# SheffieldML/GPy

Hardware: AMD Instinct MI355X
Metric: exact-GP log_lik+grad iters/sec (higher is better)
Workload: dtype f64; 1 GPU; BASELINE configs[2]: matern52 ARD exact GP, one GPRegression.parameters_changed, N=16384 D=32 Dy=1 per GPU; N=16384, D=32, kernel=matern52, ARD=True, parallelism=replicas x1

## Files before the change

gpy_amd/_lib.py:

```python
import ctypes
import os
import subprocess

import numpy as np
from numpy.ctypeslib import ndpointer

_HERE = os.path.dirname(os.path.abspath(__file__))
LIB_PATH = os.environ.get("MI355GP_LIB") or os.path.join(_HERE, "libmi355gp.so")
CSRC = os.path.join(_HERE, "csrc")

KIND_IDS = {"rbf": 0, "matern52": 1, "matern32": 2, "exponential": 3, "white": 4, "bias": 5, "ratquad": 6, "stdperiodic": 7,
            "coregionalize": 8, "linear": 9, "mlp": 10, "poly": 11, "cosine": 12, "sinc": 13, "expquadcosine": 14}


def ard_id(kind, ARD):
    if kind == "coregionalize":
        return int(ARD)
    return int(ARD) & 3 if kind == "stdperiodic" else int(bool(ARD))


class Part(ctypes.Structure):
    _fields_ = [("kind", ctypes.c_int), ("ard", ctypes.c_int), ("n_active", ctypes.c_int),
                ("active_dims", ctypes.POINTER(ctypes.c_int)), ("theta", ctypes.POINTER(ctypes.c_double)),
                ("term", ctypes.c_int)]


def make_parts(specs):
    arr = (Part * len(specs))()
    keep, ntheta = [], 0
    for i, spec in enumerate(specs):
        kind, ARD, theta, dims = spec[:4]
        arr[i].term = int(spec[4]) if len(spec) > 4 else 0
        th = np.ascontiguousarray(theta, dtype=np.float64)
        keep.append(th)
        arr[i].kind = KIND_IDS[kind]
        arr[i].ard = ard_id(kind, ARD)
        arr[i].theta = th.ctypes.data_as(ctypes.POINTER(ctypes.c_double))
        if dims is None:
            arr[i].n_active = 0
            arr[i].active_dims = None
        else:
            d = np.ascontiguousarray(dims, dtype=np.int32)
            keep.append(d)
            arr[i].n_active = d.size
            arr[i].active_dims = d.ctypes.data_as(ctypes.POINTER(ctypes.c_int))
        ntheta += th.size
    return arr, keep, ntheta
FETCH_L, FETCH_KINV, FETCH_DLDK, FETCH_K = 0, 1, 2, 3
EP_BERNOULLI_PROBIT = 0
OUT_LML, OUT_LOGDET, OUT_DATAFIT, OUT_DNOISE, OUT_TRKINV, NUM_OUT = 0, 1, 2, 3, 4, 8
STAGE_NAMES = ("kbuild", "potrf", "trtri", "lauum", "solve", "grad", "total")
NUM_T = 8
PROFILE_FAMILIES = ("update_nt", "trtri", "lauum", "diag128", "trsm128", "update_nt64", "potrf_persist", "trtri_early")

_lib = None


class MI355GPError(RuntimeError):
    pass


DIAG_LIB_PATH = os.path.join(_HERE, "libmi355gp_diag.so")


def build(force=False):
    srcs = [os.path.join(CSRC, f) for f in os.listdir(CSRC) if f.endswith((".hip", ".h")) or f == "Makefile"]
    srcs.append(os.path.join(_HERE, "..", "include", "mi355gp.h"))
    srcs.append(os.path.join(_HERE, "..", "include", "mi355gp_debug.h"))
    product = os.path.join(_HERE, "libmi355gp.so")
    if not force and os.path.exists(product) and os.path.exists(DIAG_LIB_PATH):
        t = min(os.path.getmtime(product), os.path.getmtime(DIAG_LIB_PATH))
        if all(os.path.getmtime(s) <= t for s in srcs if os.path.exists(s)):
            return product
    r = subprocess.run(["make", "-C", CSRC, "-j8", "all", "diag"], capture_output=True, text=True)
    if r.returncode != 0 or not os.path.exists(product) or not os.path.exists(DIAG_LIB_PATH):
        raise MI355GPError("building libmi355gp.so failed:\n" + r.stdout[-4000:] + r.stderr[-4000:])
    return product


_ci, _i64, _cd, _vp, _str = ctypes.c_int, ctypes.c_int64, ctypes.c_double, ctypes.c_void_p, ctypes.c_char_p
_dp = ndpointer(dtype=np.float64, flags="C_CONTIGUOUS")
_c_dp = ctypes.POINTER(ctypes.c_double)
_ip, _hp, _parts = ctypes.POINTER(_ci), ctypes.POINTER(_vp), ctypes.POINTER(Part)
_i32a, _i64a = (ndpointer(dtype=t, flags="C_CONTIGUOUS") for t in (np.int32, np.int64))
_EXACT = [_vp, _ci, _ci, _dp, _dp, _i64, _cd, _cd, _dp] + [_c_dp] * 4
_KERN_X2 = [_dp, _i64, _c_dp, _i64, _ci, _dp]

ABI = {
    "mi355gp_last_error": [],
    "mi355gp_version": [],
    "mi355gp_device_count": [_ip],
    "mi355gp_device_synchronize": [_ci],
    "mi355gp_create": [_ci, _hp],
    "mi355gp_destroy": [_vp],
    "mi355gp_set_data": [_vp, _dp, _i64, _ci, _dp, _ci],
    "mi355gp_set_targets": [_vp, _dp, _ci],
    "mi355gp_kern_K": [_ci, _ci, _ci, _dp] + _KERN_X2,
    "mi355gp_kern_Kdiag": [_ci, _dp, _i64, _dp],
    "mi355gp_update_gradients_full": [_ci, _ci, _ci, _dp, _dp] + _KERN_X2,
    "mi355gp_gradients_X": [_ci, _ci, _ci, _dp, _dp] + _KERN_X2,
    "mi355gp_exact_inference": _EXACT,
    "mi355gp_exact_inference_sum": [_vp, _ci, _parts, _dp, _i64, _cd, _cd, _dp] + [_c_dp] * 4,
    "mi355gp_exact_studentt_sum": [_vp, _ci, _parts, _cd, _cd, _cd, _dp] + [_c_dp] * 3,
    "mi355gp_inference_given_K": [_vp, _dp, _dp, _i64, _cd, _cd, _dp] + [_c_dp] * 3,
    "mi355gp_fetch": [_vp, _ci, _dp, _ci],
    "mi355gp_predict": [_vp, _ci, _ci, _dp, _dp, _i64, _c_dp, _c_dp, _ci],
    "mi355gp_predict_sum": [_vp, _ci, _parts, _dp, _i64, _c_dp, _c_dp, _ci],
    "mi355gp_predictive_gradients_sum": [_vp, _ci, _parts, _dp, _i64, _c_dp, _c_dp],
    "mi355gp_laplace_begin": [_vp, _ci, _parts],
    "mi355gp_laplace_newton": [_vp, _dp, _dp, _cd, _dp, _dp, _c_dp],
    "mi355gp_laplace_finish": [_vp, _dp, _cd, _dp, _c_dp],
    "mi355gp_laplace_gradients": [_vp, _dp, _dp, _dp],
    "mi355gp_laplace_implicit": [_vp, _dp, _dp],
    "mi355gp_laplace_predict": [_vp, _ci, _parts, _dp, _i64, _dp, _c_dp, _c_dp, _ci],
    "mi355gp_ep_recompute": [_vp, _dp, _dp, _cd, _cd, _ci, _dp, _dp, _c_dp, _c_dp],
    "mi355gp_ep_sweep": [_vp, _ci, _i64a, _dp, _cd, _cd] + [_dp] * 7 + [_c_dp],
    "mi355gp_covariance_between_points": [_vp, _ci, _parts, _dp, _i64, _dp, _i64, _dp],
    "mi355gp_potrf": [_ci, _dp, _i64, _c_dp],
    "mi355gp_pdinv": [_ci, _dp, _i64] + [_c_dp] * 4,
    "mi355gp_pdinv_full": [_ci, _dp, _i64] + [_c_dp] * 5,
    "mi355gp_set_option": [_vp, _ci, _ci],
    "mi355gp_get_option": [_vp, _ci, _ip],
    "mi355gp_get_profile": [_vp, _dp, _dp, _i32a],
    "mi355gp_grid_unique_id": [_str],
    "mi355gp_grid_create": [_ci] * 6 + [_str, _hp],
    "mi355gp_grid_destroy": [_vp],
    "mi355gp_grid_set_data": [_vp, _dp, _i64, _ci, _dp, _ci],
    "mi355gp_grid_exact_inference": _EXACT,
    "mi355gp_grid_fetch": [_vp, _ci, _dp],
    "mi355gp_grid_set_option": [_vp, _ci, _ci],
    "mi355gp_grid_get_option": [_vp, _ci, _ip],
    "mi355gp_grid_coll_log": [_vp, _ci, _dp],
    "mi355gp_sparse_create": [_ci, _hp],
    "mi355gp_sparse_destroy": [_vp],
    "mi355gp_sparse_set_data": [_vp, _dp, _i64, _ci, _dp, _ci],
    "mi355gp_vardtc_inference": _EXACT,
    "mi355gp_vardtc_inference_sum": [_vp, _ci, _parts, _dp, _i64, _dp, _i64, _cd, _dp] + [_c_dp] * 6,
    "mi355gp_sparse_set_input_variance": [_vp, _dp, _i64, _ci],
    "mi355gp_sparse_set_inputs": [_vp, _dp, _c_dp, _i64, _ci],
    "mi355gp_vardtc_inference_uncertain": [_vp, _ci, _parts, _dp, _i64, _dp, _i64, _cd, _dp] + [_c_dp] * 6,
    "mi355gp_sparse_predict": [_vp, _ci, _parts, _dp, _i64, _c_dp, _c_dp, _ci],
    "mi355gp_sparse_predict_uncertain": [_vp, _ci, _parts, _dp, _dp, _i64, _dp, _c_dp],
    "mi355gp_sparse_get_predict_ms": [_vp, _c_dp],
    "mi355gp_sparse_fetch_dLdKnm": [_vp, _i64, _i64, _dp],
    "mi355gp_sparse_attach_comm": [_vp, _ci, _ci, _str],
    "mi355gp_sparse_attach_loopback": [_vp, _ci, _ci, _ci],
    "mi355gp_sparse_fetch": [_vp, _ci, _dp],
    "mi355gp_sparse_get_profile": [_vp, _dp],
    "mi355gp_svgp_forward": [_vp, _ci, _parts, _dp, _i64, _dp, _dp, _ci, _cd, _dp, _dp, _dp, _c_dp],
    "mi355gp_svgp_backward": [_vp, _dp, _dp] + [_c_dp] * 5,
    "mi355gp_svgp_predict": [_vp, _ci, _parts, _c_dp, _i64, _ci] + [_c_dp] * 4,
    "mi355gp_pep_inference": [_vp, _ci, _parts, _dp, _i64, _cd, _cd, _cd, _dp] + [_c_dp] * 5,
    "mi355gp_pep_check_sigma": [_dp, _i64, _i64, _cd, _cd],
    "mi355gp_rbf_psi": [_ci, _cd, _dp, _ci, _dp, _i64, _dp, _dp, _i64, _ci] + [_c_dp] * 3,
    "mi355gp_rbf_psi_grad": [_ci, _cd, _dp, _ci, _dp, _i64, _dp, _dp, _i64, _ci] + [_c_dp] * 4 + [_dp] * 5,
    "mi355gp_bench_factor": [_ci, _i64, _ci, _c_dp, _c_dp, _c_dp],
    "mi355gp_dbg_ipc_selftest": [_str, _ci, _ci, _ci, _ci, _i64, _dp],
    "mi355gp_dbg_comm_selftest": [_ci, _str, _ci, _ci, _ci, _ci, _i64, _ci, _dp],
    "mi355gp_dbg_grid_multi": [_ci, _ci, _ci, _ci, _dp],
    "mi355gp_dbg_update_nt": [_ci, _ci, _ip, _ci, _ci, _dp],
    "mi355gp_dbg_update_rect": [_ci, _ci, _ci, _ip, _ci, _ci, _dp],
    "mi355gp_dbg_mfma": [_ci, _dp, _dp, _dp],
    "mi355gp_dbg_gemm": [_ci, _ci, _ci, _i64, _i64, _i64, _dp, _dp, _dp, _cd, _cd, _ci, _c_dp],
    "mi355gp_dbg_peaks": [_ci, _dp],
    "mi355gp_dbg_gemm_clock": [_c_dp, _c_dp],
    "mi355gp_dbg_cu_map": [_ci, _ci, _ci, ctypes.POINTER(ctypes.c_uint)],
    "mi355gp_dbg_pipe_share": [_ci, _dp],
    "mi355gp_dbg_graph_factor": [_ci, _i64, _ci, _dp],
    "mi355gp_dbg_persist": [_ci, _i64, _ci, _ci, _dp],
    "mi355gp_dbg_lauum_plan": [_ci, _ip, _ci, _ip],
    "mi355gp_dbg_persist_owners": [_ci, _ci, _ci, _ip, _ip],
    "mi355gp_dbg_mask_probe": [_ci, _ci, _ci, _dp],
}
EXPORTED = tuple(ABI)


def _opt(a):
    return None if a is None else a.ctypes.data_as(_c_dp)


def lib():
    global _lib
    if _lib is None:
        if not os.path.exists(LIB_PATH):
            build()
        L = ctypes.CDLL(LIB_PATH)
        for name, argtypes in ABI.items():
            getattr(L, name).argtypes = argtypes
        L.mi355gp_last_error.restype = L.mi355gp_version.restype = _str
        _lib = L
    return _lib


OPTIONS = {"profile": 0, "lookahead": 1, "tri_overlap": 2, "tri_min_nt": 3, "tri_h": 4, "tri_wgs": 5, "tri_half": 6,
           "part1_on_panel": 7, "nbo": 8, "solve_overlap": 9, "diag_excl_first": 10, "graph": 11, "persist": 12, "agg2": 13,
           "persist_test": 14, "persist_aborts": 15, "persist_skip": 16, "persist_sched": 17}


def last_error():
    return lib().mi355gp_last_error().decode()


def check(rc, what):
    if rc < 0:
        raise MI355GPError("%s failed (rc=%d): %s" % (what, rc, last_error()))
    return rc


def device_count():
    n = ctypes.c_int(0)
    lib().mi355gp_device_count(ctypes.byref(n))
    return n.value


def device_synchronize(device=0):
    require_device(device)
    check(lib().mi355gp_device_synchronize(int(device)), "mi355gp_device_synchronize")


def require_device(device=0):
    n = device_count()
    if device >= n:
        raise MI355GPError("no MI355X visible to HIP (device %d requested, %d present): the gpy_amd backend has "
                           "no CPU fallback" % (device, n))


def f64(a):
    return np.ascontiguousarray(a, dtype=np.float64)


def theta_vec(variance, lengthscale, ARD, D):
    ls = np.atleast_1d(np.asarray(lengthscale, dtype=np.float64)).ravel()
    if ARD:
        if ls.size == 1:
            ls = np.full(D, ls[0])
        assert ls.size == D, "ARD kernel needs one lengthscale per input dimension"
    else:
        assert ls.size == 1, "isotropic kernel has a single lengthscale"
    return np.concatenate([[float(np.asarray(variance).ravel()[0])], ls])


# ... 558 lines not shown

def dbg_gemm_clock():
    mhz, cyc = ctypes.c_double(0.0), ctypes.c_double(0.0)
    check(lib().mi355gp_dbg_gemm_clock(ctypes.byref(mhz), ctypes.byref(cyc)), "dbg_gemm_clock")
    return mhz.value, cyc.value


def dbg_peaks(device=0):
    require_device(device)
    out = np.zeros(8)
    check(lib().mi355gp_dbg_peaks(device, out), "dbg_peaks")
    return dict(mfma_f64_tflops=out[0], valu_f64_tflops=out[1], hbm_copy_gbs=out[2], hbm_fill_gbs=out[3],
                mfma_cycles_per_inst_1wave=out[4], shader_mhz_under_load=out[5], mfma_1wave_tflops=out[6],
                mfma_cycles_per_inst_loaded=out[7])


def dbg_grid_multi(T, nb=512, reps=3, device=0):
    require_device(device)
    out = np.zeros(5)
    check(lib().mi355gp_dbg_grid_multi(device, int(T), int(nb), int(reps), out), "mi355gp_dbg_grid_multi")
    return out


def dbg_update_nt(nt, ks, reps=5, device=0):
    require_device(device)
    ka = (ctypes.c_int * len(ks))(*[int(k) for k in ks])
    out = np.zeros(len(ks))
    check(lib().mi355gp_dbg_update_nt(device, int(nt), ka, len(ks), int(reps), out), "mi355gp_dbg_update_nt")
    return out


def dbg_update_rect(ntr, ntc, ks, reps=5, device=0):
    require_device(device)
    ka = (ctypes.c_int * len(ks))(*[int(k) for k in ks])
    out = np.zeros(len(ks))
    check(lib().mi355gp_dbg_update_rect(device, int(ntr), int(ntc), ka, len(ks), int(reps), out), "mi355gp_dbg_update_rect")
    return out


def persist_owners(nt, nw, tune=0):
    owner = (ctypes.c_int * (nt * nt))()
    out4 = (ctypes.c_int * 4)()
    dup = lib().mi355gp_dbg_persist_owners(nt, nw, tune, owner, out4)
    return np.frombuffer(owner, dtype=np.int32, count=nt * nt).reshape(nt, nt).copy(), out4[0], out4[1], out4[2], out4[3], dup


def lauum_plan(nt):
    out4 = (ctypes.c_int * 4)()
    lib().mi355gp_dbg_lauum_plan(nt, None, 0, out4)
    n = out4[0]
    buf = (ctypes.c_int * (6 * max(n, 1)))()
    check(lib().mi355gp_dbg_lauum_plan(nt, buf, n, out4), "mi355gp_dbg_lauum_plan")
    return np.frombuffer(buf, dtype=np.int32, count=6 * n).reshape(n, 6).copy(), out4[1], out4[2], out4[3]
```

gpy_amd/csrc/debug.hip:

```cpp
#include <vector>

#include "../../include/mi355gp.h"
#include "../../include/mi355gp_debug.h"
#include "internal.h"

int run_peaks(int device, double* out4);

extern "C" {

__global__ void k_count_lower_mismatch(const double* __restrict__ a, const double* __restrict__ b, long n, long ld,
                                       unsigned long long* __restrict__ count) {
    unsigned long long c = 0;
    for (long idx = (long)blockIdx.x * blockDim.x + threadIdx.x; idx < n * n; idx += (long)gridDim.x * blockDim.x) {
        const long i = idx / n, j = idx - i * n;
        if (j <= i && __double_as_longlong(a[i * ld + j]) != __double_as_longlong(b[i * ld + j])) ++c;
    }
    if (c) atomicAdd(count, c);
}

int mi355gp_dbg_persist(int device, int64_t N, int reps, int kcap, double* out) {
    ARG_CHECK(N >= 2 * NB && reps >= 1 && out, "mi355gp_dbg_persist: N >= 256, reps >= 1");
    HIP_CHECK(hipSetDevice(device));
    const long np = round_up(N, NB);
    const int nt = (int)(np / NB);
    hipStream_t st;
    if (factor_engine(device, &st, nullptr, nullptr) != 0) return -2;
    EngineShared gate(device);
    SyntheticSpd spd;
    DevBuf A, B, dStamp, dCount;
    WorkspaceGuard<2> guard;
    FactorWs& ws = guard.ws;
    hipEvent_t* e = guard.ev;
    if (int rc = spd.init(st, N)) return rc;
    HIP_CHECK(A.alloc(np * np));
    HIP_CHECK(B.alloc(np * np));
    HIP_CHECK(dStamp.alloc(32 * nt));
    HIP_CHECK(dCount.alloc(1));
    HIP_CHECK(hipMemset(dStamp, 0, sizeof(double) * 32 * nt));
    HIP_CHECK(hipMemset(dCount, 0, sizeof(double)));
    if (factor_ws_alloc(&ws, np) != 0) return -3;
    ws.tri_overlap = 0;
    if (kcap > 0) ws.persist_kcap = kcap;
    ws.persist_max_nt = 64;
    ws.persist = 1;
    if (int rc = guard.create_events()) return rc;
    for (int i = 0; i < 8 + 32 * nt; ++i) out[i] = 0.0;
    int info[4] = {0, 0, 0, 0};
    for (int mode = 0; mode < 2; ++mode) {
        double* M = mode == 0 ? (double*)B : (double*)A;
        ws.persist = mode;
        if (mode == 1 && !potrf_persist_eligible(np, &ws)) {
            mi355gp_set_error("mi355gp_dbg_persist: N = %ld is not eligible for the persistent factorisation", (long)N);
            return -1;
        }
        double acc = 0.0;
        for (int r = -1; r < reps; ++r) {
            spd.build(st, M);
// ... 152 lines not shown
    HIP_CHECK(C.alloc(n * n));
    HIP_CHECK(P.alloc(n * kmax));
    HIP_CHECK(hipMemset(C, 0, sizeof(double) * n * n));
    HIP_CHECK(hipMemset(P, 0, sizeof(double) * n * kmax));
    hipStream_t st;
    HIP_CHECK(hipStreamCreate(&st));
    hipEvent_t e0, e1;
    HIP_CHECK(hipEventCreate(&e0));
    HIP_CHECK(hipEventCreate(&e1));
    for (int i = 0; i < nk; ++i) {
        const int r0 = (ntc == ntr) ? 0 : ntc, nr = (ntc == ntr) ? ntr : ntr - ntc;
        launch_update_nt(st, C + (long)r0 * NB * n, n, P + (long)r0 * NB * kmax, kmax, P, kmax, ks[i], nr, ntc, r0, 0);
        HIP_CHECK(hipEventRecord(e0, st));
        for (int r = 0; r < reps; ++r)
            launch_update_nt(st, C + (long)r0 * NB * n, n, P + (long)r0 * NB * kmax, kmax, P, kmax, ks[i], nr, ntc, r0, 0);
        HIP_CHECK(hipEventRecord(e1, st));
        HIP_CHECK(hipEventSynchronize(e1));
        float t;
        HIP_CHECK(hipEventElapsedTime(&t, e0, e1));
        out_ms[i] = t / reps;
    }
    (void)hipEventDestroy(e0);
    (void)hipEventDestroy(e1);
    (void)hipStreamDestroy(st);
    HIP_CHECK(hipGetLastError());
    return 0;
}

int mi355gp_dbg_peaks(int device, double* out4) { return run_peaks(device, out4); }

int mi355gp_dbg_gemm_clock(double* mhz, double* cycles) { return gemm_last_clock(mhz, cycles); }

int mi355gp_dbg_lauum_plan(int nt, int* items_out, int max_items, int* out4) {
    ARG_CHECK(nt >= 1 && nt <= 4096 && out4 && (items_out || max_items == 0), "mi355gp_dbg_lauum_plan: bad arguments");
    std::vector<LauumItem> items;
    std::vector<LauumSum> sums;
    int nparts = 0;
    lauum_split_plan(nt, items, sums, &nparts);
    int longest = 0;
    for (const LauumItem& it : items) longest = it.klen > longest ? it.klen : longest;
    out4[0] = (int)items.size();
    out4[1] = nparts;
    out4[2] = lauum_split_tile(nt);
    out4[3] = longest;
    if ((int)items.size() > max_items) return -1;
    for (size_t i = 0; i < items.size(); ++i) {
        const LauumItem& it = items[i];
        const int row[6] = {it.ti, it.tj, it.q, it.k0, it.klen, it.part};
        for (int j = 0; j < 6; ++j) items_out[6 * i + j] = row[j];
    }
    return 0;
}

int mi355gp_dbg_mask_probe(int device, int pct, int order, double* out3) {
    ARG_CHECK(out3 && pct > 0 && pct <= 100, "mi355gp_dbg_mask_probe: bad arguments");
    HIP_CHECK(hipSetDevice(device));
    const long n = 4096;
    DevBuf A, B, C;
    HIP_CHECK(A.alloc(n * n));
    HIP_CHECK(B.alloc(n * n));
    HIP_CHECK(C.alloc(n * n));
    HIP_CHECK(hipMemset(A, 0, sizeof(double) * n * n));
    HIP_CHECK(hipMemset(B, 0, sizeof(double) * n * n));
    HIP_CHECK(hipMemset(C, 0, sizeof(double) * n * n));
    hipDeviceProp_t prop;
    HIP_CHECK(hipGetDeviceProperties(&prop, device));
    const int ncu = prop.multiProcessorCount, nx = 8, per = ncu / nx, keep = (per * pct + 50) / 100;
    std::vector<uint32_t> mask((size_t)(ncu + 31) / 32, 0u);
    for (int cu = 0; cu < ncu; ++cu)
        if (cu / nx < keep) mask[cu / 32] |= 1u << (cu % 32);
    int least = 0, greatest = 0;
    HIP_CHECK(hipDeviceGetStreamPriorityRange(&least, &greatest));
    hipStream_t plain = nullptr, masked = nullptr, extra[7] = {};
    auto mk_masked = [&]() { return hipExtStreamCreateWithCUMask(&masked, (uint32_t)mask.size(), mask.data()); };
    if (order == 0) {
        HIP_CHECK(mk_masked());
        HIP_CHECK(hipStreamCreate(&plain));
    } else {
        HIP_CHECK(hipStreamCreate(&plain));
        if (order == 2) {
            for (int i = 0; i < 4; ++i) HIP_CHECK(hipStreamCreateWithFlags(&extra[i], hipStreamNonBlocking));
            for (int i = 4; i < 7; ++i) HIP_CHECK(hipStreamCreateWithPriority(&extra[i], hipStreamNonBlocking, greatest));
        }
        if (order >= 1) launch_gemm(plain, 0, 1, n, n, n, A, n, B, n, C, n, 1.0, 0.0);
        HIP_CHECK(hipStreamSynchronize(plain));
        HIP_CHECK(mk_masked());
    }
    hipEvent_t e0, e1;
    HIP_CHECK(hipEventCreate(&e0));
    HIP_CHECK(hipEventCreate(&e1));
    hipStream_t order_s[3] = {plain, masked, masked};
    for (int i = 0; i < 3; ++i) {
        launch_gemm(order_s[i], 0, 1, n, n, n, A, n, B, n, C, n, 1.0, 0.0);
        HIP_CHECK(hipEventRecord(e0, order_s[i]));
        for (int r = 0; r < 3; ++r) launch_gemm(order_s[i], 0, 1, n, n, n, A, n, B, n, C, n, 1.0, 0.0);
        HIP_CHECK(hipEventRecord(e1, order_s[i]));
        HIP_CHECK(hipStreamSynchronize(order_s[i]));
        float ms = 0.f;
        HIP_CHECK(hipEventElapsedTime(&ms, e0, e1));
        out3[i] = ms / 3.0;
    }
    (void)hipEventDestroy(e0);
    (void)hipEventDestroy(e1);
    (void)hipStreamDestroy(plain);
    (void)hipStreamDestroy(masked);
    for (auto x : extra)
// ... 6 lines not shown
```

gpy_amd/csrc/gemm.hip:

```cpp
#include "gemm_tile.h"
#include "internal.h"

#define LDS_OPT_IN(kernel)                                                                              \
    do {                                                                                                \
        static bool done = false;                                                                       \
        if (!done) {                                                                                    \
            (void)hipFuncSetAttribute(reinterpret_cast<const void*>(kernel),                            \
                                      hipFuncAttributeMaxDynamicSharedMemorySize, GT_LDS_BYTES);        \
            done = true;                                                                                \
        }                                                                                               \
    } while (0)

#include <algorithm>
#include <cstdlib>
#include <vector>
#define env_int(name, dflt) diag_env_int(DIAG_ENV(name), dflt)
#define LB(NW) __launch_bounds__((NW) * 64, (NW) / 2)

template <int NW, bool PRE>
__global__ LB(NW) void k_update_nt(double* __restrict__ C, long ldc,
                                                      const double* __restrict__ A, long lda,
                                                      const double* __restrict__ B, long ldb, int K, int ntc,
                                                      int row0t, int col0t, int tri, long ntiles) {
    extern __shared__ __attribute__((aligned(16))) double smem[];
    for (long bid = blockIdx.x; bid < ntiles; bid += gridDim.x) {
        int ti, tj;
        if (tri) {
            ti = (int)((sqrtf(8.0f * (float)bid + 1.0f) - 1.0f) * 0.5f);
            while ((long)ti * (ti + 1) / 2 > bid) --ti;
            while ((long)(ti + 1) * (ti + 2) / 2 <= bid) ++ti;
            tj = (int)(bid - (long)ti * (ti + 1) / 2);
        } else {
            ti = (int)(bid / ntc);
            tj = (int)(bid - (long)ti * ntc);
            if (col0t + tj > row0t + ti) continue;
        }
        d4 acc[4][GTCfg<NW>::NI];
        double* Ct = C + (long)ti * NB * ldc + (long)tj * NB;
        if (PRE) {
            gt_load_buf<NW>(Ct, ldc, acc);
            gemm_tile_128<true, true, NW, true>(A + (long)ti * NB * lda, lda, B + (long)tj * NB * ldb, ldb, K, acc, smem);
            gt_store<0, NW>(Ct, ldc, acc);
        } else {
            gt_zero<NW>(acc);
            gemm_tile_128<true, true, NW>(A + (long)ti * NB * lda, lda, B + (long)tj * NB * ldb, ldb, K, acc, smem);
            gt_store<2, NW>(Ct, ldc, acc);
        }
    }
}

__global__ __launch_bounds__(256) void k_update_nt64(double* __restrict__ C, long ldc, const double* __restrict__ A, long lda,
                                                     const double* __restrict__ B, long ldb, int K, int ntc, int row0t,
                                                     int col0t, int tri) {
    extern __shared__ __attribute__((aligned(16))) double smem[];
// ... 194 lines not shown
    LDS_OPT_IN((k_trtri_stage<1, NW>));
    LDS_OPT_IN((k_trtri_stage<2, NW>));
    if (stages & 1)
        hipLaunchKernelGGL((k_trtri_stage<1, NW>), dim3((unsigned)nblocks), dim3(NW * 64), GT_LDS_BYTES, st, L, X, T, ld, nt, nbt);
    if (stages & 2)
        hipLaunchKernelGGL((k_trtri_stage<2, NW>), dim3((unsigned)nblocks), dim3(NW * 64), GT_LDS_BYTES, st, L, X, T, ld, nt, nbt);
}

void launch_trtri_level(hipStream_t st, const double* L, double* X, double* T, long ld, int nt, int level, int stages) {
    const int nbt = 1 << level;
    if (nbt >= nt) return;
    const long nblocks = trtri_level_tiles(nt, nbt);
    if (nblocks <= 0) return;
    static const int tri64_max = env_int("TRI64_MAX", GEMM_DEFAULT_TRI64_MAX);
    if (nblocks <= tri64_max) {
        if (stages & 1)
            hipLaunchKernelGGL((k_trtri_stage64<1>), dim3((unsigned)(4 * nblocks)), dim3(256), GT64_LDS_BYTES, st, L, X, T, ld, nt, nbt);
        if (stages & 2)
            hipLaunchKernelGGL((k_trtri_stage64<2>), dim3((unsigned)(4 * nblocks)), dim3(256), GT64_LDS_BYTES, st, L, X, T, ld, nt, nbt);
        return;
    }
    launch_trtri_level_t<4>(st, nblocks, L, X, T, ld, nt, nbt, stages);
}

template <int NW>
__global__ LB(NW) void k_lauum(const double* __restrict__ X, double* __restrict__ W, long ld, int nt) {
    extern __shared__ __attribute__((aligned(16))) double smem[];
    const int bid = blockIdx.x;
    int ti = (int)((sqrtf(8.0f * (float)bid + 1.0f) - 1.0f) * 0.5f);
    while ((long)ti * (ti + 1) / 2 > bid) --ti;
    while ((long)(ti + 1) * (ti + 2) / 2 <= bid) ++ti;
    const int tj = bid - (int)((long)ti * (ti + 1) / 2);
    d4 acc[4][GTCfg<NW>::NI];
    gt_zero<NW>(acc);
    const int K = (nt - ti) * NB;
    gemm_tile_128<false, false, NW>(X + (long)ti * NB * ld + (long)ti * NB, ld, X + (long)ti * NB * ld + (long)tj * NB, ld,
                                K, acc, smem);
    gt_store<0, NW>(W + (long)ti * NB * ld + (long)tj * NB, ld, acc);
}

__global__ __launch_bounds__(256) void k_lauum64(const double* __restrict__ X, double* __restrict__ W, long ld, int nt) {
    extern __shared__ __attribute__((aligned(16))) double smem[];
    const int bid = blockIdx.x >> 2, qi = (blockIdx.x >> 1) & 1, qj = blockIdx.x & 1;
    int ti = (int)((sqrtf(8.0f * (float)bid + 1.0f) - 1.0f) * 0.5f);
    while ((long)ti * (ti + 1) / 2 > bid) --ti;
    while ((long)(ti + 1) * (ti + 2) / 2 <= bid) ++ti;
    const int tj = bid - (int)((long)ti * (ti + 1) / 2);
    d4 acc[2][2];
    gt64_zero(acc);
    const int K = (nt - ti) * NB;
    const long r0 = (long)ti * NB + qi * 64, c0 = (long)tj * NB + qj * 64;
    gemm_tile_64_v3<false, false>(X + (long)ti * NB * ld + r0, ld, X + (long)ti * NB * ld + c0, ld, K, acc, smem);
    gt64_store<0>(W + r0 * ld + c0, ld, acc);
}

#define LAUUM_KC 1024
#define LAUUM_T128_MIN_NT 24
static int lauum_kc_rows_128(int nt) {
    static const int forced = env_int("LAUUM_KC", 0);
    if (forced >= NB) return forced / NB * NB;
    int best = LAUUM_KC;
    double best_us = 1e30;
    for (int kc = 2; kc <= 32 && kc <= nt; ++kc) {
        std::vector<int> len;
        long parts = 0;
        for (int ti = 0; ti < nt; ++ti) {
            const int K = nt - ti, nch = (K + kc - 1) / kc;
            for (int tj = 0; tj <= ti; ++tj)
                for (int c = 0; c < nch; ++c) len.push_back(c + 1 < nch ? kc : K - c * kc);
            if (nch > 1) parts += (long)nch * (ti + 1);
        }
        std::sort(len.begin(), len.end(), [](int a, int b) { return a > b; });
        std::vector<double> slot(512, 0.0);
        std::make_heap(slot.begin(), slot.end(), [](double a, double b) { return a > b; });
        double end = 0.0;
        for (int l : len) {
            std::pop_heap(slot.begin(), slot.end(), [](double a, double b) { return a > b; });
            const double t = slot.back() + 27.4 * l + 8.0;
            slot.back() = t;
            if (t > end) end = t;
            std::push_heap(slot.begin(), slot.end(), [](double a, double b) { return a > b; });
        }
        const double us = end + (double)parts * (NB * NB * 8.0) / 3.0e6;
        if (us < best_us - 0.5) {
            best_us = us;
            best = kc * NB;
        }
    }
    return best;
}
__global__ __launch_bounds__(256) void k_lauum64_items(const double* __restrict__ X, double* __restrict__ W, long ld,
                                                       const LauumItem* __restrict__ items, double* __restrict__ part) {
    extern __shared__ __attribute__((aligned(16))) double smem[];
    const LauumItem it = items[blockIdx.x];
    d4 acc[2][2];
    gt64_zero(acc);
    const long r0 = (long)it.ti * NB + (it.q >> 1) * 64, c0 = (long)it.tj * NB + (it.q & 1) * 64;
    gemm_tile_64_v3<false, false>(X + (long)it.k0 * ld + r0, ld, X + (long)it.k0 * ld + c0, ld, it.klen, acc, smem);
    if (it.part < 0) gt64_store<0>(W + r0 * ld + c0, ld, acc);
    else gt64_store<0>(part + (long)it.part * 4096, 64, acc);
}

__global__ LB(4) void k_lauum128_items(const double* __restrict__ X, double* __restrict__ W, long ld,
                                       const LauumItem* __restrict__ items, double* __restrict__ part) {
    extern __shared__ __attribute__((aligned(16))) double smem[];
    const LauumItem it = items[blockIdx.x];
// ... 20 lines not shown
__global__ __launch_bounds__(256) void k_lauum64_reduce(double* __restrict__ W, long ld, const LauumSum* __restrict__ sums,
                                                        const double* __restrict__ part) {
    const LauumSum sm = sums[blockIdx.x];
    const long r0 = (long)sm.ti * NB + (sm.q >> 1) * 64, c0 = (long)sm.tj * NB + (sm.q & 1) * 64;
    for (int e = threadIdx.x; e < 2048; e += 256) {
        const int i = e >> 5, j = 2 * (e & 31);
        d2 s = *reinterpret_cast<const d2*>(part + (long)sm.first * 4096 + i * 64 + j);
        for (int c = 1; c < sm.n; ++c) s += *reinterpret_cast<const d2*>(part + (long)(sm.first + c) * 4096 + i * 64 + j);
        *reinterpret_cast<d2*>(W + (r0 + i) * ld + c0 + j) = s;
    }
}

int lauum_split_tile(int nt) { return nt >= LAUUM_T128_MIN_NT ? 128 : 64; }

void lauum_split_plan(int nt, std::vector<LauumItem>& items, std::vector<LauumSum>& sums, int* nparts) {
    items.clear();
    sums.clear();
    int np = 0;
    const int nq = lauum_split_tile(nt) == 128 ? 1 : 4;
    static const int kc64 = env_int("LAUUM_KC64", 0) / NB * NB;
    const int kc = (nq == 1) ? lauum_kc_rows_128(nt) : (kc64 >= NB ? kc64 : (nt <= 16 ? 512 : LAUUM_KC));
    for (int ti = 0; ti < nt; ++ti)
        for (int tj = 0; tj <= ti; ++tj)
            for (int q = 0; q < nq; ++q) {
                const int k0 = ti * NB, K = (nt - ti) * NB, nch = (K + kc - 1) / kc;
                if (nch > 1) sums.push_back(LauumSum{ti, tj, q, np, nch});
                for (int c = 0; c < nch; ++c) {
                    const int len = (c + 1 < nch) ? kc : K - c * kc;
                    items.push_back(LauumItem{ti, tj, q, k0 + c * kc, len, nch > 1 ? np++ : -1});
                }
            }
    std::stable_sort(items.begin(), items.end(), [](const LauumItem& a, const LauumItem& b) { return a.klen > b.klen; });
    *nparts = np;
}

void launch_lauum_split(hipStream_t st, const double* X, double* W, long ld, int nt, const LauumItem* items_dev, int nitems,
                        const LauumSum* sums_dev, int nsums, double* part) {
    if (lauum_split_tile(nt) == 128) {
        LDS_OPT_IN(k_lauum128_items);
        hipLaunchKernelGGL(k_lauum128_items, dim3((unsigned)nitems), dim3(256), GT_LDS_BYTES, st, X, W, ld, items_dev, part);
        if (nsums > 0) hipLaunchKernelGGL(k_lauum128_reduce, dim3((unsigned)nsums), dim3(256), 0, st, W, ld, sums_dev, part);
        return;
    }
    hipLaunchKernelGGL(k_lauum64_items, dim3((unsigned)nitems), dim3(256), GT64_LDS_BYTES, st, X, W, ld, items_dev, part);
    if (nsums > 0) hipLaunchKernelGGL(k_lauum64_reduce, dim3((unsigned)nsums), dim3(256), 0, st, W, ld, sums_dev, part);
}

template <int NW>
static void launch_lauum_t(hipStream_t st, long nblocks, const double* X, double* W, long ld, int nt) {
    LDS_OPT_IN((k_lauum<NW>));
    hipLaunchKernelGGL((k_lauum<NW>), dim3((unsigned)nblocks), dim3(NW * 64), GT_LDS_BYTES, st, X, W, ld, nt);
}

bool lauum_uses_64(int nt) {
    static const int lauum64_max = env_int("LAUUM64_MAX", GEMM_DEFAULT_LAUUM64_MAX);
    return (long)nt * (nt + 1) / 2 <= lauum64_max;
}

void launch_lauum(hipStream_t st, const double* X, double* W, long ld, int nt) {
    const long nblocks = (long)nt * (nt + 1) / 2;
    static const int lauum64_max = env_int("LAUUM64_MAX", GEMM_DEFAULT_LAUUM64_MAX);
    if (nblocks <= lauum64_max) {
        hipLaunchKernelGGL(k_lauum64, dim3((unsigned)(4 * nblocks)), dim3(256), GT64_LDS_BYTES, st, X, W, ld, nt);
        return;
    }
    launch_lauum_t<4>(st, nblocks, X, W, ld, nt);
}

template <int NW>
__global__ LB(NW) void k_trmm_lower(const double* __restrict__ X, long ldx,
                                                       const double* __restrict__ B, long ldb,
                                                       double* __restrict__ Out, long ldo, int ntc) {
    extern __shared__ __attribute__((aligned(16))) double smem[];
    const int ti = (int)(gridDim.x / ntc) - 1 - (int)(blockIdx.x / ntc), tj = blockIdx.x % ntc;
    d4 acc[4][GTCfg<NW>::NI];
    gt_zero<NW>(acc);
    gemm_tile_128<true, false, NW>(X + (long)ti * NB * ldx, ldx, B + (long)tj * NB, ldb, (ti + 1) * NB, acc, smem);
    gt_store<0, NW>(Out + (long)ti * NB * ldo + (long)tj * NB, ldo, acc);
}

template <int NW>
__global__ LB(NW) void k_trmm_lower_T(const double* __restrict__ X, long ldx, const double* __restrict__ B, long ldb,
                                      double* __restrict__ Out, long ldo, int ntc, int nt) {
    extern __shared__ __attribute__((aligned(16))) double smem[];
    const int ti = blockIdx.x / ntc, tj = blockIdx.x % ntc;
    d4 acc[4][GTCfg<NW>::NI];
    gt_zero<NW>(acc);
    gemm_tile_128<false, false, NW>(X + (long)ti * NB * ldx + (long)ti * NB, ldx, B + (long)ti * NB * ldb + (long)tj * NB, ldb,
                                    (nt - ti) * NB, acc, smem);
    gt_store<0, NW>(Out + (long)ti * NB * ldo + (long)tj * NB, ldo, acc);
}

void launch_trmm_lower_T(hipStream_t st, const double* X, long ldx, const double* B, long ldb, double* Out, long ldo,
                         int ntr, int ntc) {
    LDS_OPT_IN((k_trmm_lower_T<4>));
    hipLaunchKernelGGL((k_trmm_lower_T<4>), dim3((unsigned)(ntr * ntc)), dim3(256), GT_LDS_BYTES, st, X, ldx, B, ldb, Out,
                       ldo, ntc, ntr);
}

template <int NW>
static void launch_trmm_lower_t(hipStream_t st, const double* X, long ldx, const double* B, long ldb, double* Out,
                                long ldo, int ntr, int ntc) {
    LDS_OPT_IN((k_trmm_lower<NW>));
    hipLaunchKernelGGL((k_trmm_lower<NW>), dim3((unsigned)(ntr * ntc)), dim3(NW * 64), GT_LDS_BYTES, st, X, ldx, B, ldb,
                       Out, ldo, ntc);
}

void launch_trmm_lower(hipStream_t st, const double* X, long ldx, const double* B, long ldb, double* Out, long ldo,
                       int ntr, int ntc) {
    launch_trmm_lower_t<4>(st, X, ldx, B, ldb, Out, ldo, ntr, ntc);
}

template <int MODE>
__global__ __launch_bounds__(256) void k_trmm64(const double* __restrict__ X, long ldx, const double* __restrict__ B, long ldb,
                                                double* __restrict__ Out, long ldo, int nt, int ntother, double alpha) {
    extern __shared__ __attribute__((aligned(16))) double smem[];
// ... 146 lines not shown
```

gpy_amd/csrc/gemm_tile.h:

```cpp
#pragma once
#include "common.h"

#define GT_LDS_BYTES 73728

template <int NW>
struct GTCfg {
    static_assert(NW == 4, "the tile kernels run 4-wave workgroups");
    static constexpr int NTHR = NW * 64;
    static constexpr int NI = 4;
    static constexpr int WCOLS = NI * 16;
    static constexpr int WPR = 128 / WCOLS;
};

template <bool AK, bool BK, bool NEGA = false>
__device__ __forceinline__ void gemm_tile_128_v3(const double* __restrict__ A, long lda, const double* __restrict__ B,
                                                 long ldb, int K, d4 (&acc)[4][4], double* smem);

template <bool AK, bool BK, int NW, bool NEGA = false>
__device__ __forceinline__ void gemm_tile_128(const double* __restrict__ A, long lda,
                                              const double* __restrict__ B, long ldb, int K,
                                              d4 (&acc)[4][GTCfg<NW>::NI], double* smem) {
    gemm_tile_128_v3<AK, BK, NEGA>(A, lda, B, ldb, K, acc, smem);
}

// ... 182 lines not shown
        const int r = arow + mi * 16, c = bcol + mi * 16;
        fa0[mi] = AK ? r * 16 : r;
        fb0[mi] = BK ? c * 16 : c;
    }
    const int ha = gt3_h(arow), hb = gt3_h(bcol);
    int pk = k0, ps = 0;
    const double* Ab = Atab[pk] + aoff;
    const double* Bb = Btab[pk] + boff;
    gt3_issue<AK>(rsrc(Ab), va, 0, smem, w);
    gt3_issue<BK>(rsrc(Bb), vb, 0, smem + GT3_OP, w);
    __builtin_amdgcn_s_waitcnt(0x0F70);
    __syncthreads();
    for (int kt = 0; kt < nk; ++kt) {
        const int cur = kt & 1;
        if (kt + 1 < nk) {
            if (++ps == slabs) {
                ps = 0;
                ++pk;
                Ab = Atab[pk] + aoff;
                Bb = Btab[pk] + boff;
            }
            double* nxt = smem + (cur ^ 1) * 2 * GT3_OP;
            gt3_issue<AK>(rsrc(Ab + ps * sa), va, 0, nxt, w);
            gt3_issue<BK>(rsrc(Bb + ps * sb), vb, 0, nxt + GT3_OP, w);
        }
        const double* a_s = smem + cur * 2 * GT3_OP;
        const double* b_s = a_s + GT3_OP;
#pragma unroll
        for (int e = 0; e < 2; ++e) {
            d2 af[4], bf[4];
#pragma unroll
            for (int mi = 0; mi < 4; ++mi) {
                if (AK) af[mi] = *reinterpret_cast<const d2*>(a_s + fa0[mi] + 2 * ((2 * kq + e) ^ ha));
                else af[mi] = (d2){a_s[(4 * kq + 2 * e) * GT3_SMN + fa0[mi]], a_s[(4 * kq + 2 * e + 1) * GT3_SMN + fa0[mi]]};
            }
#pragma unroll
            for (int ni = 0; ni < 4; ++ni) {
                if (BK) bf[ni] = *reinterpret_cast<const d2*>(b_s + fb0[ni] + 2 * ((2 * kq + e) ^ hb));
                else bf[ni] = (d2){b_s[(4 * kq + 2 * e) * GT3_SMN + fb0[ni]], b_s[(4 * kq + 2 * e + 1) * GT3_SMN + fb0[ni]]};
            }
#pragma unroll
            for (int s = 0; s < 2; ++s)
#pragma unroll
                for (int mi = 0; mi < 4; ++mi)
#pragma unroll
                    for (int ni = 0; ni < 4; ++ni)
                        acc[mi][ni] = mfma_f64(NEGA ? -af[mi][s] : af[mi][s], bf[ni][s], acc[mi][ni]);
        }
        __builtin_amdgcn_s_waitcnt(0x0F70);
        __syncthreads();
    }
}

#define GT64_OP 1088
#define GT64_PAIR 136
#define GT64_LDS_BYTES (2 * 2 * GT64_OP * 8)

template <bool KC>
__device__ __forceinline__ void gt64_src_offsets(long ld, int lane, int w, int (&voff)[2]) {
#pragma unroll
    for (int ii = 0; ii < 2; ++ii) {
        const int i = 2 * w + ii;
        if (KC) {
            const int row = 8 * i + (lane >> 3), g = (lane & 7) ^ gt3_h(row);
            voff[ii] = (int)((row * ld + 2 * g) * 8);
        } else {
            voff[ii] = (int)(((2 * i + (lane >> 5)) * ld + 2 * (lane & 31)) * 8);
        }
    }
}

template <bool KC>
__device__ __forceinline__ void gt64_issue(__amdgpu_buffer_rsrc_t rs, const int (&voff)[2], double* sdst, int w) {
#pragma unroll
    for (int ii = 0; ii < 2; ++ii) {
        const int i = 2 * w + ii;
        double* d = KC ? sdst + i * 128 : sdst + i * GT64_PAIR;
        __builtin_amdgcn_raw_ptr_buffer_load_lds(rs, d, 16, voff[ii], 0, 0, 0);
    }
}

template <bool AK, bool BK, bool NEGA = false>
__device__ __forceinline__ void gemm_tile_64_v3(const double* __restrict__ A, long lda, const double* __restrict__ B,
                                                long ldb, int K, d4 (&acc)[2][2], double* smem) {
    const int t = threadIdx.x, lane = t & 63, w = t >> 6, wr = w >> 1, wc = w & 1;
    const int nk = K / 16;
    const int arow = wr * 32 + (lane & 15), bcol = wc * 32 + (lane & 15), kq = lane >> 4;
    auto rsrc = [](const double* p) {
        return __builtin_amdgcn_make_buffer_rsrc(const_cast<double*>(p), 0, 0x7fffffff, 0x00020000);
    };
    int va[2], vb[2];
    gt64_src_offsets<AK>(lda, lane, w, va);
    gt64_src_offsets<BK>(ldb, lane, w, vb);
    const long sa = AK ? 16 : 16 * lda, sb = BK ? 16 : 16 * ldb;
    int fa0[2], fb0[2];
#pragma unroll
    for (int mi = 0; mi < 2; ++mi) {
        const int r = arow + mi * 16, c = bcol + mi * 16;
        fa0[mi] = AK ? r * 16 : r;
        fb0[mi] = BK ? c * 16 : c;
    }
    const int ha = gt3_h(arow), hb = gt3_h(bcol);
    gt64_issue<AK>(rsrc(A), va, smem, w);
    gt64_issue<BK>(rsrc(B), vb, smem + GT64_OP, w);
    __builtin_amdgcn_s_waitcnt(0x0F70);
    __syncthreads();
// ... 65 lines not shown
```

gpy_amd/csrc/internal.h:

```cpp
#pragma once
#include <shared_mutex>
#include <vector>

#include "common.h"

bool update_nt_uses_64(int ntr, int ntc, int row0t, int col0t);
struct UpdTask { long c_off, p_off, ntiles; int K, ntr; };
#ifdef MI355GP_DIAG
void launch_update_nt_queue(hipStream_t st, double* A, long ld, const UpdTask* tasks_dev, int ntasks, int* counter, int wgs);
#endif
void launch_update_nt(hipStream_t st, double* C, long ldc, const double* A, long lda, const double* B, long ldb,
                      int K, int ntr, int ntc, int row0t, int col0t);
void launch_trtri_level(hipStream_t st, const double* L, double* X, double* T, long ld, int nt, int level,
                        int stages = 3);
void launch_lauum(hipStream_t st, const double* X, double* W, long ld, int nt);
struct LauumItem { int ti, tj, q, k0, klen, part; };
struct LauumSum { int ti, tj, q, first, n; };
void lauum_split_plan(int nt, std::vector<LauumItem>& items, std::vector<LauumSum>& sums, int* nparts);
int lauum_split_tile(int nt);
void launch_lauum_split(hipStream_t st, const double* X, double* W, long ld, int nt, const LauumItem* items_dev, int nitems,
                        const LauumSum* sums_dev, int nsums, double* part);
bool lauum_uses_64(int nt);
void launch_trmm_lower(hipStream_t st, const double* X, long ldx, const double* B, long ldb, double* Out, long ldo,
                       int ntr, int ntc);
void launch_trmm_lower_T(hipStream_t st, const double* X, long ldx, const double* B, long ldb, double* Out, long ldo,
                         int ntr, int ntc);
void launch_trmm64(hipStream_t st, int mode, const double* X, long ldx, const double* B, long ldb, double* Out, long ldo, int nt,
                   int ntother, double alpha);
void launch_gemm_tn_sq(hipStream_t st, const double* A, long lda, long K, double* C, long ldc, int nt, double alpha,
                       double beta);
void launch_dbg_gemm(hipStream_t st, int a_mcontig, int b_ncontig, long M, long N, long K, const double* A,
                     const double* B, double* C, double alpha, double beta);

void launch_diag128(hipStream_t st, double* A, long ld, long c0, double* dinv, double* logsum, int* info,
                    int exclusive = 0);
void launch_trsm128(hipStream_t st, double* A, long ld, long c0, long r0, long mrows, const double* dinv);
void launch_trtri_stage1_steal(hipStream_t st, const double* L, double* X, double* T, long ld, int nt, int level,
                               int* counter, int grid);
void launch_inv128(hipStream_t st, const double* L, double* X, long ld, int nblk, const double* dinv_all);
void launch_dbg_mfma(hipStream_t st, const double* a, const double* b, double* d);

enum { PF_UPDATE = 0, PF_TRTRI = 1, PF_LAUUM = 2, PF_DIAG = 3, PF_TRSM = 4, PF_UPDATE64 = 5, PF_PERSIST = 6, PF_TRTRI_EARLY = 7, PF_NUM = 8 };
struct KernelProf {
    unsigned mask = 0;
    bool on = false;
    std::vector<hipEvent_t> pool;
    struct Rec { int fam; double flops; size_t e0; };
    std::vector<Rec> recs;
    bool open = false;
    void begin(hipStream_t st, int fam, double flops);
    void end(hipStream_t st);
    void reset() { recs.clear(); }
    int collect(double* ms, double* flops, int* launches);
    void destroy();
};

struct FactorWs {
    double* dinv = nullptr;
    double* logsum = nullptr;
    int* info = nullptr;
    long nblk = 0;
    hipStream_t st_panel = nullptr;
    std::vector<hipEvent_t> ev_panel;
    std::vector<hipEvent_t> ev_cols;
    hipEvent_t ev_fork = nullptr;
    hipEvent_t ev_early_pre = nullptr;
    int agg2 = 0;
    int persist_auto = 1, sched_state = 0, sched_force_steps = 0, persist_auto_off = 0;
// ... 194 lines not shown
```

Measured before the change: 14.15 iters/s.

## Add 128x256 wide-tile LAUUM kernel with triple-buffered LDS DMA pipeline

Adds a LAUUM path that computes pairs of adjacent 128-wide output tiles per workgroup using a new 128x256 MFMA f64 tile GEMM. Operands are staged into a 3-stage LDS ring via buffer_load_lds, with fragment loads interleaved into the MFMA stream. The intent is to reuse the shared A panel across two output tiles and raise arithmetic intensity for large nt (>=72, which N=16384 with nt=128 meets). The trade-off is higher register and LDS use per workgroup, at one workgroup per CU, and fewer blocks in the grid. Debug entry points for comparing the two variants are also added.

```diff
diff --git a/gpy_amd/_lib.py b/gpy_amd/_lib.py
--- a/gpy_amd/_lib.py
+++ b/gpy_amd/_lib.py
@@ -67,6 +67,7 @@
     srcs = [os.path.join(CSRC, f) for f in os.listdir(CSRC) if f.endswith((".hip", ".h")) or f == "Makefile"]
     srcs.append(os.path.join(_HERE, "..", "include", "mi355gp.h"))
     srcs.append(os.path.join(_HERE, "..", "include", "mi355gp_debug.h"))
+    srcs.append(os.path.join(_HERE, "..", "include", "mi355gp_debug_lauum.h"))
     product = os.path.join(_HERE, "libmi355gp.so")
     if not force and os.path.exists(product) and os.path.exists(DIAG_LIB_PATH):
         t = min(os.path.getmtime(product), os.path.getmtime(DIAG_LIB_PATH))
@@ -173,6 +174,10 @@
     "mi355gp_dbg_mask_probe": [_ci, _ci, _ci, _dp],
 }
 EXPORTED = tuple(ABI)
+DEBUG_LAUUM_ABI = {
+    "mi355gp_dbg_lauum_wide_map": [_ci, _ip, _ci, _ip],
+    "mi355gp_dbg_lauum": [_ci, _i64, _c_dp, _c_dp, _ci, _ci, _c_dp],
+}
 
 
 def _opt(a):
@@ -185,8 +190,9 @@
         if not os.path.exists(LIB_PATH):
             build()
         L = ctypes.CDLL(LIB_PATH)
-        for name, argtypes in ABI.items():
-            getattr(L, name).argtypes = argtypes
+        for table in (ABI, DEBUG_LAUUM_ABI):
+            for name, argtypes in table.items():
+                getattr(L, name).argtypes = argtypes
         L.mi355gp_last_error.restype = L.mi355gp_version.restype = _str
         _lib = L
     return _lib
@@ -851,3 +857,25 @@
     buf = (ctypes.c_int * (6 * max(n, 1)))()
     check(lib().mi355gp_dbg_lauum_plan(nt, buf, n, out4), "mi355gp_dbg_lauum_plan")
     return np.frombuffer(buf, dtype=np.int32, count=6 * n).reshape(n, 6).copy(), out4[1], out4[2], out4[3]
+
+
+def lauum_wide_map(nt):
+    out4 = (ctypes.c_int * 4)()
+    lib().mi355gp_dbg_lauum_wide_map(nt, None, 0, out4)
+    n = out4[0]
+    buf = (ctypes.c_int * (4 * max(n, 1)))()
+    check(lib().mi355gp_dbg_lauum_wide_map(nt, buf, n, out4), "mi355gp_dbg_lauum_wide_map")
+    return np.frombuffer(buf, dtype=np.int32, count=4 * n).reshape(n, 4).copy(), bool(out4[1]), out4[2]
+
+
+def dbg_lauum(X, variant, reps=0, device=0):
+    require_device(device)
+    ms = ctypes.c_double(0.0)
+    if isinstance(X, (int, np.integer)):
+        check(lib().mi355gp_dbg_lauum(device, int(X), None, None, int(variant), int(reps), ctypes.byref(ms)), "mi355gp_dbg_lauum")
+        return None, ms.value
+    X = f64(X)
+    W = np.zeros_like(X)
+    check(lib().mi355gp_dbg_lauum(device, X.shape[0], X.ctypes.data_as(_c_dp), W.ctypes.data_as(_c_dp), int(variant), int(reps),
+                                  ctypes.byref(ms)), "mi355gp_dbg_lauum")
+    return W, ms.value
diff --git a/gpy_amd/csrc/debug.hip b/gpy_amd/csrc/debug.hip
--- a/gpy_amd/csrc/debug.hip
+++ b/gpy_amd/csrc/debug.hip
@@ -2,7 +2,9 @@
 
 #include "../../include/mi355gp.h"
 #include "../../include/mi355gp_debug.h"
+#include "../../include/mi355gp_debug_lauum.h"
 #include "internal.h"
+#include "lauum_policy.h"
 
 int run_peaks(int device, double* out4);
 
@@ -261,6 +263,69 @@
     return 0;
 }
 
+int mi355gp_dbg_lauum_wide_map(int nt, int* items_out, int max_items, int* out4) {
+    ARG_CHECK(nt >= 1 && nt <= 4096 && out4 && (items_out || max_items == 0), "mi355gp_dbg_lauum_wide_map: bad arguments");
+    const long n = lauum_wide_items(nt);
+    int nwide = 0;
+    for (long b = 0; b < n; ++b) {
+        int ti, tj, wide;
+        lauum_wide_item(b, ti, tj, wide);
+        nwide += wide;
+        if (b < max_items) {
+            const int row[4] = {ti, tj, wide ? 2 : 1, (nt - ti) * NB};
+            for (int j = 0; j < 4; ++j) items_out[4 * b + j] = row[j];
+        }
+    }
+    out4[0] = (int)n;
+    out4[1] = lauum_wide_applies(nt, 0) ? 1 : 0;
+    out4[2] = LAUUM_WIDE_MIN_NT;
+    out4[3] = nwide;
+    return n > max_items ? -1 : 0;
+}
+
+__global__ void k_dbg_fill_lower(double* __restrict__ X, long n) {
+    for (long idx = (long)blockIdx.x * blockDim.x + threadIdx.x; idx < n * n; idx += (long)gridDim.x * blockDim.x) {
+        const long i = idx / n, j = idx - i * n;
+        unsigned long long h = (unsigned long long)idx * 0x9E3779B97F4A7C15ull;
+        h ^= h >> 29;
+        h *= 0xBF58476D1CE4E5B9ull;
+        h ^= h >> 32;
+        X[idx] = j <= i ? (double)(h >> 11) * (2.0 / 9007199254740992.0) - 1.0 : 0.0;
+    }
+}
+
+int mi355gp_dbg_lauum(int device, int64_t n, const double* X_host, double* W_host, int variant, int reps, double* ms) {
+    ARG_CHECK(n >= NB && n % NB == 0 && n <= 65536 && (variant == 0 || variant == 1) && reps >= 0 && (reps == 0 || ms),
+              "mi355gp_dbg_lauum: n a multiple of 128, variant 0 or 1, reps >= 0");
+    HIP_CHECK(hipSetDevice(device));
+    const int nt = (int)(n / NB);
+    DevBuf X, W;
+    HIP_CHECK(X.alloc(n * n));
+    HIP_CHECK(W.alloc(n * n));
+    if (X_host) HIP_CHECK(hipMemcpy(X, X_host, sizeof(double) * n * n, hipMemcpyHostToDevice));
+    else hipLaunchKernelGGL(k_dbg_fill_lower, dim3(4096), dim3(256), 0, 0, (double*)X, (long)n);
+    HIP_CHECK(hipMemset(W, 0, sizeof(double) * n * n));
+    launch_lauum_variant(0, X, W, n, nt, variant);
+    HIP_CHECK(hipDeviceSynchronize());
+    if (W_host) HIP_CHECK(hipMemcpy(W_host, W, sizeof(double) * n * n, hipMemcpyDeviceToHost));
+    if (reps > 0) {
+        hipEvent_t e0, e1;
+        HIP_CHECK(hipEventCreate(&e0));
+        HIP_CHECK(hipEventCreate(&e1));
+        HIP_CHECK(hipEventRecord(e0, 0));
+        for (int r = 0; r < reps; ++r) launch_lauum_variant(0, X, W, n, nt, variant);
+        HIP_CHECK(hipEventRecord(e1, 0));
+        HIP_CHECK(hipEventSynchronize(e1));
+        float t;
+        HIP_CHECK(hipEventElapsedTime(&t, e0, e1));
+        *ms = t / reps;
+        (void)hipEventDestroy(e0);
+        (void)hipEventDestroy(e1);
+    }
+    HIP_CHECK(hipGetLastError());
+    return 0;
+}
+
 int mi355gp_dbg_mask_probe(int device, int pct, int order, double* out3) {
     ARG_CHECK(out3 && pct > 0 && pct <= 100, "mi355gp_dbg_mask_probe: bad arguments");
     HIP_CHECK(hipSetDevice(device));
diff --git a/gpy_amd/csrc/gemm.hip b/gpy_amd/csrc/gemm.hip
--- a/gpy_amd/csrc/gemm.hip
+++ b/gpy_amd/csrc/gemm.hip
@@ -1,5 +1,6 @@
 #include "gemm_tile.h"
 #include "internal.h"
+#include "lauum_policy.h"
 
 #define LDS_OPT_IN(kernel)                                                                              \
     do {                                                                                                \
@@ -300,6 +301,27 @@
     const long r0 = (long)ti * NB + qi * 64, c0 = (long)tj * NB + qj * 64;
     gemm_tile_64_v3<false, false>(X + (long)ti * NB * ld + r0, ld, X + (long)ti * NB * ld + c0, ld, K, acc, smem);
     gt64_store<0>(W + r0 * ld + c0, ld, acc);
+}
+
+__global__ __launch_bounds__(256, 1) void k_lauum_wide(const double* __restrict__ X, double* __restrict__ W, long ld, int nt) {
+    extern __shared__ __attribute__((aligned(16))) double smem[];
+    int ti, tj, wide;
+    lauum_wide_item((long)blockIdx.x, ti, tj, wide);
+    const int K = (nt - ti) * NB;
+    const double* Ap = X + (long)ti * NB * ld + (long)ti * NB;
+    const double* Bp = X + (long)ti * NB * ld + (long)tj * NB;
+    double* Wp = W + (long)ti * NB * ld + (long)tj * NB;
+    if (wide) {
+        d4 acc[8][4];
+        gtw_zero(acc);
+        gemm_tile_128x256<false, false>(Ap, ld, Bp, ld, K, acc, smem);
+        gtw_store(Wp, ld, acc);
+    } else {
+        d4 acc[4][GTCfg<4>::NI];
+        gt_zero<4>(acc);
+        gemm_tile_128<false, false, 4>(Ap, ld, Bp, ld, K, acc, smem);
+        gt_store<0, 4>(Wp, ld, acc);
+    }
 }
 
 #define LAUUM_KC 1024
@@ -426,6 +448,21 @@
     hipLaunchKernelGGL((k_lauum<NW>), dim3((unsigned)nblocks), dim3(NW * 64), GT_LDS_BYTES, st, X, W, ld, nt);
 }
 
+static void launch_lauum_wide(hipStream_t st, const double* X, double* W, long ld, int nt) {
+    static bool done = false;
+    if (!done) {
+        (void)hipFuncSetAttribute(reinterpret_cast<const void*>(k_lauum_wide), hipFuncAttributeMaxDynamicSharedMemorySize,
+                                  GTW_LDS_BYTES);
+        done = true;
+    }
+    hipLaunchKernelGGL(k_lauum_wide, dim3((unsigned)lauum_wide_items(nt)), dim3(256), GTW_LDS_BYTES, st, X, W, ld, nt);
+}
+
+void launch_lauum_variant(hipStream_t st, const double* X, double* W, long ld, int nt, int variant) {
+    if (variant) launch_lauum_wide(st, X, W, ld, nt);
+    else launch_lauum_t<4>(st, (long)nt * (nt + 1) / 2, X, W, ld, nt);
+}
+
 bool lauum_uses_64(int nt) {
     static const int lauum64_max = env_int("LAUUM64_MAX", GEMM_DEFAULT_LAUUM64_MAX);
     return (long)nt * (nt + 1) / 2 <= lauum64_max;
@@ -436,6 +473,11 @@
     static const int lauum64_max = env_int("LAUUM64_MAX", GEMM_DEFAULT_LAUUM64_MAX);
     if (nblocks <= lauum64_max) {
         hipLaunchKernelGGL(k_lauum64, dim3((unsigned)(4 * nblocks)), dim3(256), GT64_LDS_BYTES, st, X, W, ld, nt);
+        return;
+    }
+    static const int wide_on = env_int("LAUUM_WIDE", 1);
+    if (lauum_wide_applies(nt, !wide_on)) {
+        launch_lauum_wide(st, X, W, ld, nt);
         return;
     }
     launch_lauum_t<4>(st, nblocks, X, W, ld, nt);
diff --git a/gpy_amd/csrc/gemm_tile.h b/gpy_amd/csrc/gemm_tile.h
--- a/gpy_amd/csrc/gemm_tile.h
+++ b/gpy_amd/csrc/gemm_tile.h
@@ -258,6 +258,91 @@
     }
 }
 
+#define GTW_S 388
+#define GTW_STAGE (16 * GTW_S)
+#define GTW_LDS_BYTES (3 * GTW_STAGE * 8)
+
+template <bool AK, bool BK>
+__device__ __forceinline__ void gemm_tile_128x256(const double* __restrict__ A, long lda, const double* __restrict__ B,
+                                                  long ldb, int K, d4 (&acc)[8][4], double* smem) {
+    static_assert(!AK && !BK, "gemm_tile_128x256: only the TN form (both operands m/n-contiguous) is built");
+    const int t = threadIdx.x, lane = t & 63, w = __builtin_amdgcn_readfirstlane(t >> 6), kq = lane >> 4;
+    const int nk = K / 16;
+    auto rsrc = [](const double* p) {
+        return __builtin_amdgcn_make_buffer_rsrc(const_cast<double*>(p), 0, 0x7fffffff, 0x00020000);
+    };
+    const int voff = lane * 16;
+    const int lda8 = (int)lda * 8, ldb8 = (int)ldb * 8;
+    auto dma = [&](__amdgpu_buffer_rsrc_t ra, __amdgpu_buffer_rsrc_t rb, int stage, int i) {
+        const int kr = 4 * w + i / 3, pc = i % 3;
+        double* d = smem + stage * GTW_STAGE + kr * GTW_S + pc * 128;
+        if (pc == 0) __builtin_amdgcn_raw_ptr_buffer_load_lds(ra, d, 16, voff, kr * lda8, 0, 0);
+        else __builtin_amdgcn_raw_ptr_buffer_load_lds(rb, d, 16, voff, kr * ldb8 + (pc - 1) * 1024, 0, 0);
+    };
+    auto slab_a = [&](int slab) { return rsrc(A + (long)(slab < nk ? slab : nk - 1) * 16 * lda); };
+    auto slab_b = [&](int slab) { return rsrc(B + (long)(slab < nk ? slab : nk - 1) * 16 * ldb); };
+    const int fbase = 4 * kq * GTW_S + (lane & 15);
+    auto frag = [&](const double* p, int u, d2 (&af)[8], d2 (&bf)[4]) {
+        if (u < 8) af[u] = (d2){p[u * 16], p[GTW_S + u * 16]};
+        else bf[u - 8] = (d2){p[128 + 64 * w + (u - 8) * 16], p[GTW_S + 128 + 64 * w + (u - 8) * 16]};
+    };
+    d2 a0[8], b0[4], a1[8], b1[4];
+#pragma unroll
+    for (int sl = 0; sl < 3; ++sl) {
+        const __amdgpu_buffer_rsrc_t ra = slab_a(sl), rb = slab_b(sl);
+#pragma unroll
+        for (int i = 0; i < 12; ++i) dma(ra, rb, sl, i);
+    }
+    __builtin_amdgcn_s_waitcnt(0x4F78);
+    __builtin_amdgcn_s_barrier();
+#pragma unroll
+    for (int u = 0; u < 12; ++u) frag(smem + fbase, u, a0, b0);
+    int cur = 0;
+    for (int kt = 0; kt < nk; ++kt) {
+        const int nxt = cur == 2 ? 0 : cur + 1;
+        const double* p1 = smem + cur * GTW_STAGE + fbase + 2 * GTW_S;
+#pragma unroll
+        for (int i = 0; i < 64; ++i) {
+            const int s = i >> 5, mi = (i >> 2) & 7, ni = i & 3;
+            acc[mi][ni] = mfma_f64(a0[mi][s], b0[ni][s], acc[mi][ni]);
+            if (i < 12) frag(p1, i, a1, b1);
+            __builtin_amdgcn_sched_barrier(0);
+        }
+        __builtin_amdgcn_s_waitcnt(0x007C);
+        __builtin_amdgcn_s_barrier();
+        const __amdgpu_buffer_rsrc_t ra = slab_a(kt + 3), rb = slab_b(kt + 3);
+        const double* p0 = smem + nxt * GTW_STAGE + fbase;
+#pragma unroll
+        for (int i = 0; i < 64; ++i) {
+            const int s = i >> 5, mi = (i >> 2) & 7, ni = i & 3;
+            acc[mi][ni] = mfma_f64(a1[mi][s], b1[ni][s], acc[mi][ni]);
+            if (i < 12) dma(ra, rb, cur, i);
+            else if (i < 24) frag(p0, i - 12, a0, b0);
+            __builtin_amdgcn_sched_barrier(0);
+        }
+        cur = nxt;
+    }
+    __builtin_amdgcn_s_waitcnt(0x0F70);
+}
+
+__device__ __forceinline__ void gtw_zero(d4 (&acc)[8][4]) {
+#pragma unroll
+    for (int mi = 0; mi < 8; ++mi)
+#pragma unroll
+        for (int ni = 0; ni < 4; ++ni) acc[mi][ni] = (d4){0.0, 0.0, 0.0, 0.0};
+}
+
+__device__ __forceinline__ void gtw_store(double* __restrict__ C, long ldc, const d4 (&acc)[8][4]) {
+    const int t = threadIdx.x, lane = t & 63, w = t >> 6;
+    double* base = C + (long)(lane >> 4) * ldc + 64 * w + (lane & 15);
+#pragma unroll
+    for (int mi = 0; mi < 8; ++mi)
+#pragma unroll
+        for (int ni = 0; ni < 4; ++ni)
+#pragma unroll
+            for (int r = 0; r < 4; ++r) base[(long)(mi * 16 + 4 * r) * ldc + ni * 16] = acc[mi][ni][r];
+}
+
 #define GT64_OP 1088
 #define GT64_PAIR 136
 #define GT64_LDS_BYTES (2 * 2 * GT64_OP * 8)
diff --git a/gpy_amd/csrc/internal.h b/gpy_amd/csrc/internal.h
--- a/gpy_amd/csrc/internal.h
+++ b/gpy_amd/csrc/internal.h
@@ -14,6 +14,7 @@
 void launch_trtri_level(hipStream_t st, const double* L, double* X, double* T, long ld, int nt, int level,
                         int stages = 3);
 void launch_lauum(hipStream_t st, const double* X, double* W, long ld, int nt);
+void launch_lauum_variant(hipStream_t st, const double* X, double* W, long ld, int nt, int variant);
 struct LauumItem { int ti, tj, q, k0, klen, part; };
 struct LauumSum { int ti, tj, q, first, n; };
 void lauum_split_plan(int nt, std::vector<LauumItem>& items, std::vector<LauumSum>& sums, int* nparts);
diff --git a/gpy_amd/csrc/lauum_policy.h b/gpy_amd/csrc/lauum_policy.h
--- /dev/null
+++ b/gpy_amd/csrc/lauum_policy.h
@@ -0,0 +1,31 @@
+#pragma once
+#include <math.h>
+
+#ifdef __HIPCC__
+#define LAUUM_POLICY_HD __host__ __device__
+#else
+#define LAUUM_POLICY_HD
+#endif
+
+#define LAUUM_WIDE_MIN_NT 72
+
+static inline bool lauum_wide_applies(int nt, int force_old) { return !force_old && nt >= LAUUM_WIDE_MIN_NT; }
+
+LAUUM_POLICY_HD static inline long lauum_wide_items(int nt) {
+    const long m = nt / 2;
+    return (nt & 1) ? (m + 1) * (m + 1) : m * (m + 1);
+}
+
+LAUUM_POLICY_HD static inline void lauum_wide_item(long b, int& ti, int& tj, int& wide) {
+    long m = (long)((sqrtf(4.0f * (float)b + 1.0f) - 1.0f) * 0.5f);
+    while (m * (m + 1) > b) --m;
+    while ((m + 1) * (m + 2) <= b) ++m;
+    long r = b - m * (m + 1);
+    ti = (int)(2 * m);
+    if (r > m) {
+        r -= m + 1;
+        ++ti;
+    }
+    tj = (int)(2 * r);
+    wide = (tj + 1 <= ti) ? 1 : 0;
+}
diff --git a/include/mi355gp_debug_lauum.h b/include/mi355gp_debug_lauum.h
--- /dev/null
+++ b/include/mi355gp_debug_lauum.h
@@ -0,0 +1,14 @@
+#ifndef MI355GP_DEBUG_LAUUM_H
+#define MI355GP_DEBUG_LAUUM_H
+#include <stdint.h>
+#ifdef __cplusplus
+extern "C" {
+#endif
+
+int mi355gp_dbg_lauum_wide_map(int nt, int* items, int max_items, int* out4);
+int mi355gp_dbg_lauum(int device, int64_t n, const double* X, double* W, int variant, int reps, double* ms);
+
+#ifdef __cplusplus
+}
+#endif
+#endif
```

Result: faster. 14.30 iters/s (median of 6 runs) (+1.1%).
